# elrodrigues/deneva-plus

Hardware: AMD Instinct MI355X
Metric: committed txns/sec (node) YCSB zipf0.9 at 1/2/4/8 GPUs; abort-set bit-exact (higher is better)
Workload: dtype u64; 1 GPU; YCSB config D: 16,777,216 rows/partition, 1,048,576-txn epoch in total; cc_alg=NO_WAIT, rows_per_partition=16777216, txns_per_epoch=1048576, txns_per_epoch_per_gpu=1048576, req_per_query=10, parallelism=1 GPU, decision_lanes=4, sequence_order=one origin

## Files before the change

deneva-plus_amd/csrc/dvcc_prefix.hip:

```cpp
#include <algorithm>

#include "dvcc_common.h"

namespace dvcc {

namespace {
#ifndef DVCC_KILL_IPT
#define DVCC_KILL_IPT 2
#endif
constexpr int kKillIPT = DVCC_KILL_IPT;
constexpr uint32_t kKillTile = kBlock * kKillIPT;
constexpr uint32_t RS_RD = 1u, RS_WR = 2u;

__device__ __forceinline__ uint32_t row_bits(const uint32_t *rs, uint32_t row) {
    return (rs[row >> 4] >> ((row & 15u) * 2u)) & 3u;
}
}

#ifndef DVCC_HOT_LOG
#define DVCC_HOT_LOG 16
#endif
#ifndef DVCC_BLOOM_LOG
#define DVCC_BLOOM_LOG 20
#endif
constexpr uint32_t kHotRows = 1u << DVCC_HOT_LOG, kHotWords = kHotRows / 16;
constexpr uint32_t kBloomBits = 1u << DVCC_BLOOM_LOG, kBloomWords = kBloomBits / 32;
static_assert((kHotWords + kBloomWords) * sizeof(uint32_t) <= 160u * 1024u,
              "k_kill's hot row words + Bloom filter exceed gfx950's 160 KiB of LDS per workgroup");
__device__ __forceinline__ uint32_t bloom_bit(uint32_t row) { return (row * 0x9E3779B1u) >> (32 - DVCC_BLOOM_LOG); }

uint64_t row_state_words(uint64_t rows) { return (((rows + 15) / 16 + 3) & ~3ull) + kBloomWords; }

#ifndef DVCC_MARK_BLOCK
#define DVCC_MARK_BLOCK 512
#endif
constexpr int kMarkBlock = DVCC_MARK_BLOCK;
__global__ __launch_bounds__(kMarkBlock) void k_prefix_mark(uint8_t *__restrict__ status,
                                                            const uint32_t *__restrict__ tb_start,
                                                            const uint32_t *__restrict__ tb_end,
                                                            const uint32_t *__restrict__ acc_row, RecRows rr,
                                                            uint32_t K, uint32_t *__restrict__ row_state,
                                                            uint64_t state_words,
                                                            uint32_t *__restrict__ bloom, int nowait,
                                                            Counters *__restrict__ ctr,
                                                            const uint32_t *__restrict__ words) {
    __shared__ uint32_t s_hot[kHotWords];
    if (input_err(ctr)) return;
    if (ctr->halt) {
        if (blockIdx.x == 0 && threadIdx.x == 0) ctr->a_halt = 1u;
        return;
    }
    if (blockIdx.x == 0 && threadIdx.x == 0) {
        const uint32_t r0 = ctr->async_wr0 ? ctr->async_wr0 : ctr->async_r0;
        ctr->a_rounds = r0 ? r0 + ctr->async_iters : 1u;
    }
    for (uint32_t i = threadIdx.x; i < kHotWords; i += kMarkBlock) s_hot[i] = 0;
    __syncthreads();
    uint32_t und = 0;
    for (uint32_t t = blockIdx.x * kMarkBlock + threadIdx.x; t < K; t += gridDim.x * kMarkBlock) {
        if (words) {
            const uint8_t st = word_status(words[t]);
            status[t] = st;
            und += st == ST_UNDEC ? 1u : 0u;
            if (st != ST_COMMIT) continue;
        } else if (status[t] != ST_COMMIT) {
            continue;
        }
        constexpr uint32_t kMU = 8;
        for (uint32_t a0 = tb_start[t], e = tb_end[t]; a0 < e; a0 += kMU) {
            uint32_t arw[kMU];
#pragma unroll
            for (uint32_t u = 0; u < kMU; u++) arw[u] = a0 + u < e ? row_word(acc_row, rr, a0 + u) : 0u;
#pragma unroll
            for (uint32_t u = 0; u < kMU; u++) {
                if (a0 + u >= e) continue;
                const uint32_t ar = arw[u];
                const uint32_t row = ar & ~AR_WR;
                const uint32_t bit = (ar & AR_WR) ? RS_WR : (nowait ? RS_RD : 0u);
                if (!bit) continue;
                if (row < kHotRows) {
                    atomicOr(&s_hot[row >> 4], bit << ((row & 15u) * 2u));
                } else {
                    atomicOr(&row_state[row >> 4], bit << ((row & 15u) * 2u));
                    const uint32_t h = bloom_bit(row);
                    atomicOr(&bloom[h >> 5], 1u << (h & 31u));
                }
            }
        }
    }
    if (und) {
        set_err(ctr, ERRB_SPIN);
        atomicMax(&ctr->spin_site, 2u);
    }
    __syncthreads();
    for (uint32_t i = threadIdx.x; i < kHotWords && i < state_words; i += kMarkBlock) {
        const uint32_t w = s_hot[i];
        if (w) atomicOr(&row_state[i], w);
    }
}

#ifndef DVCC_KILL_WORDS
#define DVCC_KILL_WORDS 8
#endif
constexpr int kKillWords = DVCC_KILL_WORDS;
constexpr int kKillBlock = 1024;
template <int KEYS>
__global__ __launch_bounds__(kKillBlock) void k_kill(const uint32_t *__restrict__ acc_row, uint64_t n,
                                                 const uint32_t *__restrict__ n_dev,
                                                 const uint32_t *__restrict__ row_state, uint64_t state_words,
                                                 const uint32_t *__restrict__ bloom, int nowait,
                                                 uint64_t *__restrict__ kill_bits, uint64_t *__restrict__ skip_bits,
                                                 Counters *__restrict__ ctr, KillKeys kk) {
    __shared__ __align__(16) uint32_t s_lds[kHotWords + kBloomWords];
    uint32_t *const s_hot = s_lds, *const s_bloom = s_lds + kHotWords;
    if (input_err(ctr) || ctr->halt) return;
    if (n_dev && (uint64_t)*n_dev < n) n = *n_dev;
    {
        constexpr uint32_t kH4 = kHotWords / 4, kAll4 = (kHotWords + kBloomWords) / 4;
        static_assert(kAll4 % kKillBlock == 0, "k_kill's LDS fill: whole 16-byte steps per thread");
        constexpr uint32_t kSteps = kAll4 / kKillBlock;
        const uint32_t sw4 = (uint32_t)(state_words / 4 < kH4 ? state_words / 4 : kH4);
        const uint4 *hot4 = reinterpret_cast<const uint4 *>(row_state);
        const uint4 *blm4 = reinterpret_cast<const uint4 *>(bloom);
        uint4 v[kSteps];
#pragma unroll
        for (uint32_t k = 0; k < kSteps; k++) {
            const uint32_t i = k * kKillBlock + threadIdx.x;
            v[k] = i < kH4 ? (i < sw4 ? hot4[i] : make_uint4(0u, 0u, 0u, 0u)) : blm4[i - kH4];
        }
        uint4 *dst = reinterpret_cast<uint4 *>(s_lds);
#pragma unroll
        for (uint32_t k = 0; k < kSteps; k++) dst[k * kKillBlock + threadIdx.x] = v[k];
    }
    __syncthreads();
    const uint64_t first = ctr->a_acc;
    const uint32_t lane = threadIdx.x & 63;
    const uint64_t w0 = first >> 6, nw = (n + 63) >> 6;
    const uint64_t waves = (uint64_t)gridDim.x * (kKillBlock / 64);
    const uint64_t wstep = waves * kKillWords;
    auto states = [&](const uint32_t *ar, uint32_t *sw) {
#pragma unroll
        for (int q = 0; q < kKillWords; q++) {
            sw[q] = 0;
            if (ar[q] != ~0u) {
                const uint32_t row = ar[q] & ~AR_WR;
                if (row < kHotRows) {
                    sw[q] = s_hot[row >> 4];
                } else {
                    const uint32_t h = bloom_bit(row);
                    if ((s_bloom[h >> 5] >> (h & 31u)) & 1u) sw[q] = row_state[row >> 4];
                }
            }
        }
    };
    auto verdicts = [&](uint64_t w, const uint32_t *ar, const uint32_t *sw) {
#pragma unroll
        for (int q = 0; q < kKillWords; q++) {
            bool kill = false, skip = false;
            if (ar[q] != ~0u) {
                const uint32_t row = ar[q] & ~AR_WR;
                const uint32_t st = (sw[q] >> ((row & 15u) * 2u)) & 3u;
                kill = (st & RS_WR) || (nowait && st && (ar[q] & AR_WR));
                skip = st == RS_RD && !(ar[q] & AR_WR);
            }
            const uint64_t m = __ballot(kill), sm = __ballot(skip);
            if (lane == 0 && w + q < nw) {
                kill_bits[w + q] = m;
                if (skip_bits) skip_bits[w + q] = sm;
            }
        }
    };
    const uint64_t wbeg = w0 + ((uint64_t)blockIdx.x * (kKillBlock / 64) + (threadIdx.x >> 6)) * kKillWords;
    if (KEYS == 0 || (KEYS == 2 && kk.recs)) {
        const uint32_t *src = KEYS == 0 ? acc_row : kk.recs;
        uint32_t nxt[kKillWords];
        auto load = [&](uint64_t w) {
#pragma unroll
            for (int q = 0; q < kKillWords; q++) {
                const uint64_t i = ((w + q) << 6) + lane;
                nxt[q] = w < nw && i >= first && i < n ? src[i] : ~0u;
            }
        };
        load(wbeg);
        for (uint64_t w = wbeg; w < nw; w += wstep) {
            uint32_t ar[kKillWords], sw[kKillWords];
#pragma unroll
            for (int q = 0; q < kKillWords; q++) {
                ar[q] = nxt[q];
                if constexpr (KEYS == 2) {
                    const uint64_t i = ((w + q) << 6) + lane;
                    if (i >= first && i < n) {
                        const uint32_t key = nxt[q] & 0x7FFFFFFFu;
                        if (key < kk.dense_lim) {
                            ar[q] = (uint32_t)(key + kk.dense_base) | (nxt[q] & AR_WR);
                        } else {
                            set_err(ctr, ERRB_KEY);
                            ar[q] = ~0u;
                        }
                    } else {
                        ar[q] = ~0u;
                    }
                }
            }
            states(ar, sw);
            load(w + wstep);
            verdicts(w, ar, sw);
        }
        return;
    }
    for (uint64_t w = wbeg; w < nw; w += wstep) {
        uint32_t ar[kKillWords], sw[kKillWords];
        if constexpr (KEYS != 0) {
            uint64_t key[kKillWords];
            uint32_t wr[kKillWords];
            bool in[kKillWords];
#pragma unroll
            for (int q = 0; q < kKillWords; q++) {
                const uint64_t i = ((w + q) << 6) + lane;
                in[q] = i >= first && i < n;
                wr[q] = 0;
                key[q] = in[q] ? kk_key(kk, i, wr[q]) : 0ull;
            }
#pragma unroll
            for (int q = 0; q < kKillWords; q++) {
                uint64_t row = 0;
                ar[q] = ~0u;
                if (in[q] && kk_row<KEYS == 2>(kk, key[q], row, ctr))
                    ar[q] = (uint32_t)row | (wr[q] ? AR_WR : 0u);
            }
        }
        states(ar, sw);
        verdicts(w, ar, sw);
    }
}

__device__ __forceinline__ bool range_killed(const uint64_t *__restrict__ kill_bits, uint32_t a0, uint32_t a1) {
    if (a0 >= a1) return false;
    const uint32_t wlo = a0 >> 6, whi = (a1 - 1) >> 6;
    uint64_t lo = kill_bits[wlo], hi = kill_bits[whi];
    lo &= ~0ull << (a0 & 63);
    hi &= ~0ull >> (63 - ((a1 - 1) & 63));
    if (wlo == whi) return (lo & hi) != 0;
    bool k = (lo | hi) != 0;
    for (uint32_t w = wlo + 1; w < whi; w++) k |= kill_bits[w] != 0;
    return k;
}

__device__ __forceinline__ uint32_t range_count(const uint64_t *__restrict__ bits, uint32_t a0, uint32_t a1) {
    if (a0 >= a1) return 0u;
    const uint32_t wlo = a0 >> 6, whi = (a1 - 1) >> 6;
    uint64_t lo = bits[wlo] & (~0ull << (a0 & 63));
    const uint64_t hmask = ~0ull >> (63 - ((a1 - 1) & 63));
    if (wlo == whi) return (uint32_t)__popcll(lo & hmask);
    uint32_t c = (uint32_t)__popcll(lo) + (uint32_t)__popcll(bits[whi] & hmask);
    for (uint32_t w = wlo + 1; w < whi; w++) c += (uint32_t)__popcll(bits[w]);
    return c;
}

__device__ __forceinline__ uint32_t range_field(const uint64_t *__restrict__ bits, uint32_t a0, uint32_t a1) {
    if (a0 >= a1) return 0u;
    const uint32_t wlo = a0 >> 6, whi = (a1 - 1) >> 6, sh = a0 & 63u, len = a1 - a0;
    uint64_t f = bits[wlo] >> sh;
    if (whi != wlo) f |= bits[whi] << (64u - sh);
    return (uint32_t)f & (len >= 32u ? ~0u : (1u << len) - 1u);
}

__device__ __forceinline__ uint32_t nth_kept(const uint64_t *__restrict__ skip, uint32_t a0, uint32_t r) {
    uint32_t w = a0 >> 6;
    uint64_t m = ~skip[w] & (~0ull << (a0 & 63));
    for (uint32_t c = (uint32_t)__popcll(m); r >= c; c = (uint32_t)__popcll(m)) {
        r -= c;
        m = ~skip[++w];
    }
    for (; r; r--) m &= m - 1;
    return (w << 6) + (uint32_t)__builtin_ctzll(m);
}

__global__ __launch_bounds__(kBlock) void k_kill_count(const uint32_t *__restrict__ tb_start,
                                                       const uint32_t *__restrict__ tb_end, uint32_t K,
                                                       uint32_t n_txn, const uint64_t *__restrict__ kill_bits,
                                                       const uint64_t *__restrict__ skip_bits,
                                                       uint8_t *__restrict__ status, uint32_t *__restrict__ info,
                                                       uint32_t *__restrict__ tsum, const Counters *ctr) {
    __shared__ uint32_t lds4[4];
    const uint32_t m = n_txn > K ? n_txn - K : 0u;
    const uint32_t ntiles = (m + kKillTile - 1) / kKillTile;
    if (blockIdx.x >= ntiles || input_err(ctr) || ctr->halt) return;
    const uint32_t tid = threadIdx.x;
    const uint32_t t_lo = K + blockIdx.x * kKillTile;
    uint32_t a0[kKillIPT], a1[kKillIPT];
#pragma unroll
    for (int j = 0; j < kKillIPT; j++) {
        const uint32_t t = t_lo + j * kBlock + tid;
        a0[j] = t < n_txn ? tb_start[t] : 0u;
        a1[j] = t < n_txn ? tb_end[t] : 0u;
    }
    uint32_t cnt = 0, acc = 0;
#pragma unroll
    for (int j = 0; j < kKillIPT; j++) {
        const uint32_t t = t_lo + j * kBlock + tid;
        if (t >= n_txn) continue;
        const bool killed = range_killed(kill_bits, a0[j], a1[j]);
        if (killed) status[t] = ST_ABORT;
        const uint32_t len = killed ? 0u : a1[j] - a0[j] - (skip_bits ? range_count(skip_bits, a0[j], a1[j]) : 0u);
        info[t - K] = killed ? 0u : len | 0x80000000u;
        cnt += killed ? 0u : 1u;
        acc += len;
    }
    uint32_t tc = 0, ta = 0;
    (void)block_excl_scan256(cnt, lds4, &tc);
    (void)block_excl_scan256(acc, lds4, &ta);
    if (tid == 0) {
        tsum[2 * blockIdx.x] = tc;
        tsum[2 * blockIdx.x + 1] = ta;
    }
}

template <int KEYS>
__global__ __launch_bounds__(kBlock) void k_kill_emit(
    const uint32_t *__restrict__ tb_start, const uint32_t *__restrict__ tb_end, uint32_t *__restrict__ acc_row,
    uint32_t K, uint32_t n_txn,
    const uint64_t *__restrict__ skip_bits, const uint32_t *__restrict__ info, const uint32_t *__restrict__ tsum,
    uint32_t *__restrict__ map,
    uint8_t *__restrict__ status_b, uint8_t *__restrict__ tlen_b, uint64_t *__restrict__ pairs_b, Counters *ctr,
    KillKeys kk, const uint32_t *__restrict__ row_state, int nowait) {
    __shared__ Agg wt_c[kBlock / 64], wt_a[kBlock / 64], wt_f[kBlock / 64];
    __shared__ uint32_t s_sub0, s_ab0, s_nsurv, s_nacc, s_nfull;
    __shared__ uint32_t l_a0[kKillTile], l_pre[kKillTile + 1];
    __shared__ uint32_t l_st[kKillTile], l_len[kKillTile];
    __shared__ uint32_t l_end[KEYS ? kKillTile : 1], l_fl[KEYS ? kKillTile : 1], l_skip[KEYS ? kKillTile : 1];
    __shared__ uint32_t l_fpre[KEYS == 1 ? kKillTile + 1 : 1];
    const uint32_t m = n_txn > K ? n_txn - K : 0u;
    const uint32_t ntiles = (m + kKillTile - 1) / kKillTile;
    if (blockIdx.x >= ntiles || input_err(ctr) || ctr->halt) return;
    const uint32_t tid = threadIdx.x, lane = tid & 63, wave = tid >> 6;
    const uint32_t tile = blockIdx.x;
    const uint32_t t_lo = K + tile * kKillTile;
#pragma unroll
    for (int j = 0; j < kKillIPT; j++) {
        const uint32_t t = t_lo + j * kBlock + tid;
        l_st[j * kBlock + tid] = t < n_txn ? tb_start[t] : 0u;
        l_len[j * kBlock + tid] = t < n_txn ? info[t - K] : 0u;
        if constexpr (KEYS) l_end[j * kBlock + tid] = t < n_txn ? tb_end[t] : 0u;
    }
    if (wave < 2) {
        uint32_t sum = 0;
        for (uint32_t q0 = 0; q0 < tile; q0 += 8 * 64) {
            uint32_t v[8];
#pragma unroll
            for (uint32_t u = 0; u < 8; u++) {
                const uint32_t q = q0 + u * 64 + lane;
                v[u] = q < tile ? tsum[2 * q + wave] : 0u;
            }
#pragma unroll
            for (uint32_t u = 0; u < 8; u++) sum += v[u];
        }
#pragma unroll
        for (int off = 32; off > 0; off >>= 1) sum += __shfl_xor(sum, off, 64);
        if (lane == 0) {
            (wave == 0 ? s_sub0 : s_ab0) = sum;
            if (tile == ntiles - 1) (wave == 0 ? ctr->b_txn : ctr->b_acc) = sum + tsum[2 * tile + wave];
        }
    }
    __syncthreads();
    const uint32_t first = t_lo + tid * kKillIPT;
    uint32_t surv = 0, cnt = 0, acc = 0, full = 0;
    uint32_t a0s[kKillIPT], lens[kKillIPT], fls[kKillIPT];
#pragma unroll
    for (int j = 0; j < kKillIPT; j++) {
        const uint32_t w = l_len[tid * kKillIPT + j];
        a0s[j] = l_st[tid * kKillIPT + j];
        lens[j] = w & 0x7FFFFFFFu;
        fls[j] = KEYS ? l_end[tid * kKillIPT + j] - a0s[j] : 0u;
        if (!w) continue;
        surv |= 1u << j;
        cnt++;
        acc += lens[j];
        full += fls[j];
    }
    const Agg inc_c = wave_incl<OpPlain>(Agg{0u, 0u, cnt}, lane);
    const Agg inc_a = wave_incl<OpPlain>(Agg{0u, 0u, acc}, lane);
    const Agg inc_f = KEYS == 1 ? wave_incl<OpPlain>(Agg{0u, 0u, full}, lane) : Agg{0u, 0u, 0u};
    if (lane == 63) {
        wt_c[wave] = inc_c;
        wt_a[wave] = inc_a;
        wt_f[wave] = inc_f;
    }
    __syncthreads();
    if (tid == 0) {
        uint32_t c = 0, a = 0, f = 0;
        for (int w = 0; w < kBlock / 64; w++) {
            c += wt_c[w].c;
            a += wt_a[w].c;
            f += wt_f[w].c;
        }
        s_nsurv = c;
        s_nacc = a;
        s_nfull = f;
    }
    uint32_t ls = 0, la = 0, lf = 0;
    for (uint32_t w = 0; w < wave; w++) {
        ls += wt_c[w].c;
        la += wt_a[w].c;
        lf += wt_f[w].c;
    }
    ls += wave_excl_from_incl<OpPlain>(inc_c, lane).c;
    la += wave_excl_from_incl<OpPlain>(inc_a, lane).c;
    if constexpr (KEYS == 1) lf += wave_excl_from_incl<OpPlain>(inc_f, lane).c;
    __syncthreads();
    const uint32_t sub0 = s_sub0;
#pragma unroll
    for (int j = 0; j < kKillIPT; j++) {
        if (!((surv >> j) & 1u)) continue;
        const uint32_t sub = sub0 + ls;
        map[sub] = first + j;
        tlen_b[sub] = (uint8_t)lens[j];
        status_b[sub] = ST_UNDEC;
        l_a0[ls] = a0s[j];
        l_pre[ls] = la;
        if constexpr (KEYS) l_fl[ls] = fls[j];
        if constexpr (KEYS == 1) {
            l_fpre[ls] = lf;
            l_skip[ls] = 0;
        }
        if constexpr (KEYS == 2)
            l_skip[ls] = skip_bits && fls[j] <= 32u ? range_field(skip_bits, a0s[j], a0s[j] + fls[j]) : 0u;
        la += lens[j];
        lf += fls[j];
        ls++;
    }
    if (tid == 0) {
        l_pre[s_nsurv] = s_nacc;
        if constexpr (KEYS == 1) l_fpre[s_nsurv] = s_nfull;
    }
    __syncthreads();
    if constexpr (KEYS == 1) {
        constexpr uint32_t kU = 4;
        const uint32_t ns = s_nsurv, nf = s_nfull;
        for (uint32_t g0 = 0; g0 < nf; g0 += kBlock * kU) {
            uint32_t a[kU], wr[kU];
            uint64_t key[kU];
#pragma unroll
            for (uint32_t u = 0; u < kU; u++) {
                const uint32_t g = g0 + u * kBlock + tid;
                uint32_t lo = 0, hi = ns;
                while (hi - lo > 1) {
                    const uint32_t mid = (lo + hi) >> 1;
                    if (l_fpre[mid] <= g) lo = mid;
                    else hi = mid;
                }
                a[u] = l_a0[lo] + (g - l_fpre[lo]);
                wr[u] = 0;
                key[u] = g < nf ? kk_key(kk, a[u], wr[u]) : 0ull;
            }
            uint32_t rows[kU];
#pragma unroll
            for (uint32_t u = 0; u < kU; u++) {
                uint64_t row = 0;
                if (g0 + u * kBlock + tid < nf)
                    kk_row<false>(kk, key[u], row, ctr);
                rows[u] = (uint32_t)row;
            }
#pragma unroll
            for (uint32_t u = 0; u < kU; u++) {
                const uint32_t g = g0 + u * kBlock + tid;
                if (g >= nf) continue;
                acc_row[a[u]] = rows[u] | (wr[u] ? AR_WR : 0u);
#ifdef DVCC_EMIT_ROW_STATE
                const bool skip = nowait && !wr[u] && row_bits(row_state, rows[u]) == RS_RD;
#else
                const bool skip = skip_bits && ((skip_bits[a[u] >> 6] >> (a[u] & 63u)) & 1ull) != 0;
#endif
                if (skip) {
                    uint32_t lo = 0, hi = ns;
                    while (hi - lo > 1) {
                        const uint32_t mid = (lo + hi) >> 1;
                        if (l_fpre[mid] <= g) lo = mid;
                        else hi = mid;
                    }
                    if (l_fpre[lo + 1] - l_fpre[lo] <= 32u) atomicOr(&l_skip[lo], 1u << (g - l_fpre[lo]));
                }
            }
        }
        __syncthreads();
    }
    constexpr uint32_t kCompactU = 4;
    const uint32_t ns = s_nsurv, na = s_nacc, ab0 = s_ab0;
    for (uint32_t g0 = 0; g0 < na; g0 += kBlock * kCompactU) {
        uint32_t sv[kCompactU], qv[kCompactU], ar[kCompactU];
#pragma unroll
        for (uint32_t u = 0; u < kCompactU; u++) {
            const uint32_t g = g0 + u * kBlock + tid;
            uint32_t lo = 0, hi = ns;
            while (hi - lo > 1) {
                const uint32_t mid = (lo + hi) >> 1;
                if (l_pre[mid] <= g) lo = mid;
                else hi = mid;
            }
            sv[u] = lo;
            qv[u] = g - l_pre[lo];
            uint32_t a = 0;
            if (g < na) {
                if constexpr (KEYS) {
                    if (l_fl[lo] <= 32u) {
                        uint32_t kept = ~l_skip[lo];
                        for (uint32_t r = qv[u]; r; r--) kept &= kept - 1;
                        a = l_a0[lo] + (uint32_t)__builtin_ctz(kept);
                    } else {
                        a = skip_bits ? nth_kept(skip_bits, l_a0[lo], qv[u]) : l_a0[lo] + qv[u];
                    }
                } else {
                    a = skip_bits ? nth_kept(skip_bits, l_a0[lo], qv[u]) : l_a0[lo] + qv[u];
                }
            }
            if constexpr (KEYS) {
                uint64_t row = 0;
                uint32_t w = 0;
                if (g < na) kk_row<KEYS == 2>(kk, kk_key(kk, a, w), row, ctr);
                ar[u] = g < na ? (uint32_t)row | (w ? AR_WR : 0u) : 0u;
            } else {
                ar[u] = g < na ? acc_row[a] : 0u;
            }
        }
#pragma unroll
        for (uint32_t u = 0; u < kCompactU; u++) {
            const uint32_t g = g0 + u * kBlock + tid;
            if (g < na) pairs_b[ab0 + g] = pair_pack(ar[u] & ~AR_WR, sub0 + sv[u], qv[u], ar[u] >> 31);
        }
    }
}

__global__ __launch_bounds__(kBlock) void k_sub_scatter_back(const uint32_t *__restrict__ map,
                                                             const uint8_t *__restrict__ status_b,
                                                             uint8_t *__restrict__ status, Counters *ctr,
                                                             const uint32_t *__restrict__ words) {
    if (input_err(ctr) || ctr->halt) return;
    const uint32_t S = ctr->b_txn;
    uint32_t und = 0;
    for (uint32_t i = blockIdx.x * kBlock + threadIdx.x; i < S; i += gridDim.x * kBlock) {
        const uint8_t st = words ? word_status(words[i]) : status_b[i];
        status[map[i]] = st;
        und += st == ST_UNDEC ? 1u : 0u;
    }
    if (und) {
        set_err(ctr, ERRB_SPIN);
        atomicMax(&ctr->spin_site, 2u);
    }
}

namespace {
uint32_t grid_of(uint64_t n, uint32_t cap) {
    const uint64_t g = (n + kBlock - 1) / kBlock;
    return (uint32_t)(g < 1 ? 1 : (g > cap ? cap : g));
}
}

void launch_prefix_mark(hipStream_t s, uint8_t *status, const uint32_t *tb_start, const uint32_t *tb_end,
                        const uint32_t *acc_row, const RecRows &rr, uint32_t K, uint32_t *row_state,
                        uint64_t rs_words, int nowait, Counters *ctr, const uint32_t *words) {
    const uint32_t g = std::max<uint32_t>(1, std::min<uint32_t>((K + kMarkBlock - 1) / kMarkBlock, 64));
    DV_LAUNCH(k_prefix_mark, g, kMarkBlock, 0, s, status, tb_start, tb_end, acc_row, rr, K, row_state,
              rs_words - kBloomWords, row_state + (rs_words - kBloomWords), nowait, ctr, words);
}

uint32_t kill_tiles(uint32_t n_after) { return (n_after + kKillTile - 1) / kKillTile; }

uint64_t kill_words(uint64_t n_acc) { return (n_acc + 63) / 64 + 1; }

void launch_kill_compact(hipStream_t s, const uint32_t *tb_start, const uint32_t *tb_end, const uint32_t *acc_row,
                         uint64_t n_acc, const uint32_t *n_acc_dev, uint32_t K, uint32_t n_txn,
                         const uint32_t *row_state, uint64_t rs_words,
                         int nowait,
                         uint64_t *kill_bits, uint64_t *skip_bits, uint8_t *status, uint32_t *map,
                         uint8_t *status_b, uint8_t *tlen_b, uint64_t *pairs_b, uint32_t *info, uint32_t *tsum,
                         Counters *ctr, const KillKeys *kk) {
    const uint32_t nt = kill_tiles(n_txn > K ? n_txn - K : 0u);
    if (!nt) return;
    const uint64_t nw = (n_acc + 63) / 64;
    const KillKeys k0 = kk ? *kk : KillKeys{};
    uint32_t *ar = const_cast<uint32_t *>(acc_row);
    const uint32_t kg = grid_of(nw * 64 / kKillWords / 4 + 1, 256);
    if (kk && k0.dense_lim)
        DV_LAUNCH(k_kill<2>, kg, kKillBlock, 0, s, acc_row, n_acc, n_acc_dev, row_state, rs_words - kBloomWords,
                  row_state + (rs_words - kBloomWords), nowait, kill_bits, skip_bits, ctr, k0);
    else if (kk)
        DV_LAUNCH(k_kill<1>, kg, kKillBlock, 0, s, acc_row, n_acc, n_acc_dev, row_state, rs_words - kBloomWords,
                  row_state + (rs_words - kBloomWords), nowait, kill_bits, skip_bits, ctr, k0);
    else
        DV_LAUNCH(k_kill<0>, kg, kKillBlock, 0, s, acc_row, n_acc, n_acc_dev, row_state, rs_words - kBloomWords,
                  row_state + (rs_words - kBloomWords), nowait, kill_bits, skip_bits, ctr, k0);
    DV_LAUNCH(k_kill_count, nt, kBlock, 0, s, tb_start, tb_end, K, n_txn, (const uint64_t *)kill_bits,
              (const uint64_t *)skip_bits, status, info, tsum, ctr);
    if (kk && k0.dense_lim)
        DV_LAUNCH(k_kill_emit<2>, nt, kBlock, 0, s, tb_start, tb_end, ar, K, n_txn, (const uint64_t *)skip_bits,
                  info, tsum, map, status_b, tlen_b, pairs_b, ctr, k0, row_state, nowait);
    else if (kk)
        DV_LAUNCH(k_kill_emit<1>, nt, kBlock, 0, s, tb_start, tb_end, ar, K, n_txn, (const uint64_t *)skip_bits,
                  info, tsum, map, status_b, tlen_b, pairs_b, ctr, k0, row_state, nowait);
    else
        DV_LAUNCH(k_kill_emit<0>, nt, kBlock, 0, s, tb_start, tb_end, ar, K, n_txn, (const uint64_t *)skip_bits,
                  info, tsum, map, status_b, tlen_b, pairs_b, ctr, k0, row_state, nowait);
}

void launch_sub_scatter_back(hipStream_t s, const uint32_t *map, const uint8_t *status_b, uint32_t ub,
                             uint8_t *status, Counters *ctr, const uint32_t *words) {
    if (!ub) return;
    DV_LAUNCH(k_sub_scatter_back, grid_of(ub, 2048), kBlock, 0, s, map, status_b, status, ctr, words);
}

}
```

Baseline: 170.4 million committed txns/s.

## Restructure k_kill: prefetch records before LDS fill, branchless LDS lookups, batched ballot stores

The k_kill kernel now reads its counters once into scalar registers and issues the first record prefetch before the LDS fill, so global load latency overlaps the table copy. Row-state allocation is padded to at least the hot-table size, which removes the bounds check in the fill and allows an unconditional vector load. The state lookup is split into a branchless LDS read (hot word or Bloom word), a gather from global memory taken only on a Bloom hit, and a verdict pass. Each group of kKillWords ballot results is kept in per-lane registers and written by several lanes at once instead of serially by lane 0. The changes add clamped out-of-range loads and a slightly larger row_state allocation for small tables.

```diff
diff --git a/deneva-plus_amd/csrc/dvcc_prefix.hip b/deneva-plus_amd/csrc/dvcc_prefix.hip
--- a/deneva-plus_amd/csrc/dvcc_prefix.hip
+++ b/deneva-plus_amd/csrc/dvcc_prefix.hip
@@ -29,7 +29,9 @@
               "k_kill's hot row words + Bloom filter exceed gfx950's 160 KiB of LDS per workgroup");
 __device__ __forceinline__ uint32_t bloom_bit(uint32_t row) { return (row * 0x9E3779B1u) >> (32 - DVCC_BLOOM_LOG); }
 
-uint64_t row_state_words(uint64_t rows) { return (((rows + 15) / 16 + 3) & ~3ull) + kBloomWords; }
+uint64_t row_state_words(uint64_t rows) {
+    return std::max<uint64_t>(((rows + 15) / 16 + 3) & ~3ull, kHotWords) + kBloomWords;
+}
 
 #ifndef DVCC_MARK_BLOCK
 #define DVCC_MARK_BLOCK 512
@@ -104,91 +106,100 @@
 #endif
 constexpr int kKillWords = DVCC_KILL_WORDS;
 constexpr int kKillBlock = 1024;
+#ifndef DVCC_KILL_GRID
+#define DVCC_KILL_GRID 256
+#endif
 template <int KEYS>
 __global__ __launch_bounds__(kKillBlock) void k_kill(const uint32_t *__restrict__ acc_row, uint64_t n,
                                                  const uint32_t *__restrict__ n_dev,
-                                                 const uint32_t *__restrict__ row_state, uint64_t state_words,
+                                                 const uint32_t *__restrict__ row_state,
                                                  const uint32_t *__restrict__ bloom, int nowait,
                                                  uint64_t *__restrict__ kill_bits, uint64_t *__restrict__ skip_bits,
                                                  Counters *__restrict__ ctr, KillKeys kk) {
     __shared__ __align__(16) uint32_t s_lds[kHotWords + kBloomWords];
-    uint32_t *const s_hot = s_lds, *const s_bloom = s_lds + kHotWords;
-    if (input_err(ctr) || ctr->halt) return;
-    if (n_dev && (uint64_t)*n_dev < n) n = *n_dev;
+    const uint32_t err = ctr->err | ctr->peer_err, halt = ctr->halt, a_acc = ctr->a_acc;
+    const uint32_t n_real = *(n_dev ? n_dev : &ctr->a_acc);
+    asm volatile("" ::"s"(err), "s"(halt), "s"(a_acc), "s"(n_real));
+    if ((err & ERRB_INPUT) || halt) return;
+    if (n_dev && (uint64_t)n_real < n) n = n_real;
+    if (!n) return;
+    const uint64_t first = a_acc;
+    const uint32_t lane = threadIdx.x & 63;
+    const uint64_t w0 = first >> 6, nw = (n + 63) >> 6;
+    const uint64_t waves = (uint64_t)gridDim.x * (kKillBlock / 64);
+    const uint64_t wstep = waves * kKillWords;
+    const uint64_t wbeg = w0 + ((uint64_t)blockIdx.x * (kKillBlock / 64) + (threadIdx.x >> 6)) * kKillWords;
+    const bool rec_loop = KEYS == 0 || (KEYS == 2 && kk.recs);
+    const uint32_t *src = KEYS == 0 ? acc_row : kk.recs;
+    uint32_t nxt[kKillWords];
+    auto load = [&](uint64_t w) {
+#pragma unroll
+        for (int q = 0; q < kKillWords; q++) {
+            const uint64_t i = ((w + q) << 6) + lane;
+            nxt[q] = src[i < n ? i : n - 1];
+        }
+    };
+    if (rec_loop) load(wbeg);
     {
         constexpr uint32_t kH4 = kHotWords / 4, kAll4 = (kHotWords + kBloomWords) / 4;
         static_assert(kAll4 % kKillBlock == 0, "k_kill's LDS fill: whole 16-byte steps per thread");
         constexpr uint32_t kSteps = kAll4 / kKillBlock;
-        const uint32_t sw4 = (uint32_t)(state_words / 4 < kH4 ? state_words / 4 : kH4);
         const uint4 *hot4 = reinterpret_cast<const uint4 *>(row_state);
         const uint4 *blm4 = reinterpret_cast<const uint4 *>(bloom);
         uint4 v[kSteps];
 #pragma unroll
         for (uint32_t k = 0; k < kSteps; k++) {
             const uint32_t i = k * kKillBlock + threadIdx.x;
-            v[k] = i < kH4 ? (i < sw4 ? hot4[i] : make_uint4(0u, 0u, 0u, 0u)) : blm4[i - kH4];
+            v[k] = *(i < kH4 ? hot4 + i : blm4 + (i - kH4));
         }
         uint4 *dst = reinterpret_cast<uint4 *>(s_lds);
 #pragma unroll
         for (uint32_t k = 0; k < kSteps; k++) dst[k * kKillBlock + threadIdx.x] = v[k];
     }
     __syncthreads();
-    const uint64_t first = ctr->a_acc;
-    const uint32_t lane = threadIdx.x & 63;
-    const uint64_t w0 = first >> 6, nw = (n + 63) >> 6;
-    const uint64_t waves = (uint64_t)gridDim.x * (kKillBlock / 64);
-    const uint64_t wstep = waves * kKillWords;
-    auto states = [&](const uint32_t *ar, uint32_t *sw) {
+    auto lds_words = [&](const uint32_t *ar, uint32_t *lw) {
 #pragma unroll
         for (int q = 0; q < kKillWords; q++) {
-            sw[q] = 0;
-            if (ar[q] != ~0u) {
-                const uint32_t row = ar[q] & ~AR_WR;
-                if (row < kHotRows) {
-                    sw[q] = s_hot[row >> 4];
-                } else {
-                    const uint32_t h = bloom_bit(row);
-                    if ((s_bloom[h >> 5] >> (h & 31u)) & 1u) sw[q] = row_state[row >> 4];
-                }
-            }
+            const uint32_t row = ar[q] & ~AR_WR;
+            const uint32_t idx = row < kHotRows ? row >> 4 : kHotWords + (bloom_bit(row) >> 5);
+            lw[q] = s_lds[ar[q] != ~0u ? idx : 0u];
         }
     };
-    auto verdicts = [&](uint64_t w, const uint32_t *ar, const uint32_t *sw) {
+    auto gathers = [&](const uint32_t *ar, const uint32_t *lw, uint32_t *gw) {
 #pragma unroll
         for (int q = 0; q < kKillWords; q++) {
-            bool kill = false, skip = false;
-            if (ar[q] != ~0u) {
-                const uint32_t row = ar[q] & ~AR_WR;
-                const uint32_t st = (sw[q] >> ((row & 15u) * 2u)) & 3u;
-                kill = (st & RS_WR) || (nowait && st && (ar[q] & AR_WR));
-                skip = st == RS_RD && !(ar[q] & AR_WR);
-            }
-            const uint64_t m = __ballot(kill), sm = __ballot(skip);
-            if (lane == 0 && w + q < nw) {
-                kill_bits[w + q] = m;
-                if (skip_bits) skip_bits[w + q] = sm;
-            }
+            const uint32_t row = ar[q] & ~AR_WR;
+            gw[q] = 0;
+            if (ar[q] != ~0u && row >= kHotRows && ((lw[q] >> (bloom_bit(row) & 31u)) & 1u))
+                gw[q] = row_state[row >> 4];
         }
     };
-    const uint64_t wbeg = w0 + ((uint64_t)blockIdx.x * (kKillBlock / 64) + (threadIdx.x >> 6)) * kKillWords;
-    if (KEYS == 0 || (KEYS == 2 && kk.recs)) {
-        const uint32_t *src = KEYS == 0 ? acc_row : kk.recs;
-        uint32_t nxt[kKillWords];
-        auto load = [&](uint64_t w) {
+    auto verdicts = [&](uint64_t w, const uint32_t *ar, const uint32_t *lw, const uint32_t *gw) {
+        uint64_t km = 0, sm = 0;
+#pragma unroll
+        for (int q = 0; q < kKillWords; q++) {
+            const uint32_t row = ar[q] & ~AR_WR;
+            const uint32_t sw = row < kHotRows ? lw[q] : gw[q];
+            const uint32_t st = (sw >> ((row & 15u) * 2u)) & 3u;
+            const bool kill = (st & RS_WR) || (nowait && st && (ar[q] & AR_WR));
+            const bool skip = st == RS_RD && !(ar[q] & AR_WR);
+            const uint64_t m = __ballot(kill), s = __ballot(skip);
+            km = lane == (uint32_t)q ? m : km;
+            sm = lane == (uint32_t)q ? s : sm;
+        }
+        if (lane < (uint32_t)kKillWords && w + lane < nw) {
+            kill_bits[w + lane] = km;
+            if (skip_bits) skip_bits[w + lane] = sm;
+        }
+    };
+    if (rec_loop) {
+        for (uint64_t w = wbeg; w < nw; w += wstep) {
+            uint32_t ar[kKillWords], lw[kKillWords], gw[kKillWords];
 #pragma unroll
             for (int q = 0; q < kKillWords; q++) {
                 const uint64_t i = ((w + q) << 6) + lane;
-                nxt[q] = w < nw && i >= first && i < n ? src[i] : ~0u;
-            }
-        };
-        load(wbeg);
-        for (uint64_t w = wbeg; w < nw; w += wstep) {
-            uint32_t ar[kKillWords], sw[kKillWords];
-#pragma unroll
-            for (int q = 0; q < kKillWords; q++) {
-                ar[q] = nxt[q];
+                ar[q] = i >= first && i < n ? nxt[q] : ~0u;
                 if constexpr (KEYS == 2) {
-                    const uint64_t i = ((w + q) << 6) + lane;
                     if (i >= first && i < n) {
                         const uint32_t key = nxt[q] & 0x7FFFFFFFu;
                         if (key < kk.dense_lim) {
@@ -202,14 +213,15 @@
                     }
                 }
             }
-            states(ar, sw);
+            lds_words(ar, lw);
+            gathers(ar, lw, gw);
             load(w + wstep);
-            verdicts(w, ar, sw);
+            verdicts(w, ar, lw, gw);
         }
         return;
     }
     for (uint64_t w = wbeg; w < nw; w += wstep) {
-        uint32_t ar[kKillWords], sw[kKillWords];
+        uint32_t ar[kKillWords], lw[kKillWords], gw[kKillWords];
         if constexpr (KEYS != 0) {
             uint64_t key[kKillWords];
             uint32_t wr[kKillWords];
@@ -229,8 +241,9 @@
                     ar[q] = (uint32_t)row | (wr[q] ? AR_WR : 0u);
             }
         }
-        states(ar, sw);
-        verdicts(w, ar, sw);
+        lds_words(ar, lw);
+        gathers(ar, lw, gw);
+        verdicts(w, ar, lw, gw);
     }
 }
 
@@ -579,15 +592,15 @@
     const uint64_t nw = (n_acc + 63) / 64;
     const KillKeys k0 = kk ? *kk : KillKeys{};
     uint32_t *ar = const_cast<uint32_t *>(acc_row);
-    const uint32_t kg = grid_of(nw * 64 / kKillWords / 4 + 1, 256);
+    const uint32_t kg = grid_of(nw * 64 / kKillWords / 4 + 1, DVCC_KILL_GRID);
     if (kk && k0.dense_lim)
-        DV_LAUNCH(k_kill<2>, kg, kKillBlock, 0, s, acc_row, n_acc, n_acc_dev, row_state, rs_words - kBloomWords,
+        DV_LAUNCH(k_kill<2>, kg, kKillBlock, 0, s, acc_row, n_acc, n_acc_dev, row_state,
                   row_state + (rs_words - kBloomWords), nowait, kill_bits, skip_bits, ctr, k0);
     else if (kk)
-        DV_LAUNCH(k_kill<1>, kg, kKillBlock, 0, s, acc_row, n_acc, n_acc_dev, row_state, rs_words - kBloomWords,
+        DV_LAUNCH(k_kill<1>, kg, kKillBlock, 0, s, acc_row, n_acc, n_acc_dev, row_state,
                   row_state + (rs_words - kBloomWords), nowait, kill_bits, skip_bits, ctr, k0);
     else
-        DV_LAUNCH(k_kill<0>, kg, kKillBlock, 0, s, acc_row, n_acc, n_acc_dev, row_state, rs_words - kBloomWords,
+        DV_LAUNCH(k_kill<0>, kg, kKillBlock, 0, s, acc_row, n_acc, n_acc_dev, row_state,
                   row_state + (rs_words - kBloomWords), nowait, kill_bits, skip_bits, ctr, k0);
     DV_LAUNCH(k_kill_count, nt, kBlock, 0, s, tb_start, tb_end, K, n_txn, (const uint64_t *)kill_bits,
               (const uint64_t *)skip_bits, status, info, tsum, ctr);
```

Result: faster. 175.6 million committed txns/s, median of 6 (+3.1%).
